# palash1992/GEM

Measured on NVIDIA H100. Metric: nodes/sec embedded at d=128, higher is better.
Workload: dtype f32

## Files before the change

### gem_b200/csrc/common.cuh

```cuda
#pragma once
#include <cuda_runtime.h>
#include <stdint.h>
#include <stdio.h>
#include <string>
#include <vector>
#include "../../include/gemb200.h"

namespace gemb {

void set_error(const char *fmt, ...);
void count_launch(int k = 1);

#define GEMB_CUDA(call)                                                                       \
    do {                                                                                      \
        cudaError_t _e = (call);                                                              \
        if (_e != cudaSuccess) {                                                              \
            gemb::set_error("%s failed at %s:%d: %s", #call, __FILE__, __LINE__,              \
                            cudaGetErrorString(_e));                                          \
            (void)cudaGetLastError();           \
            return GEMB_ERR_CUDA;                                                             \
        }                                                                                     \
    } while (0)

#define GEMB_TRY(call)                                                                        \
// ... 51 lines not shown
    float ms(int from, int to) const { float t = 0.f; cudaEventElapsedTime(&t, ev_[from], ev_[to]); return t; }

  private:
    cudaEvent_t ev_[N] = {};
};

struct Timer {
    std::vector<cudaEvent_t> ev;
    size_t used = 0;
    int begin(cudaStream_t s);
    int end(cudaStream_t s);
    double total_ms();
    void reset() { used = 0; }
    void destroy();
};

}

struct gemb_halo_pool {
    size_t cap_floats = 0;
    int nbuf = 0;
    float *buf[8] = {};
    float *peer_buf[8][8] = {};
    unsigned long long *flags = nullptr;
    unsigned long long *peer_flags[8] = {};
    unsigned long long epoch = 0;
    int *timeout_flag = nullptr;
};

struct gemb_ctx {
    int device = 0;
    int sm_count = 132;
    cudaStream_t stream = nullptr;
    int rank = 0, nranks = 1;
    void *comm = nullptr;
    float *spmm_scratch = nullptr;
    size_t spmm_scratch_bytes = 0;
    double *red_scratch = nullptr;
    size_t red_scratch_bytes = 0;
    gemb::Timer t_spmm, t_dense, t_comm, t_misc;
    gemb_halo_pool halo_pool;
};

struct gemb_csr_dev {
    int64_t nnz = 0;
    int32_t *indptr = nullptr;
    int32_t *indices = nullptr;
    float *data = nullptr;
    int32_t n_heavy = 0, n_items = 0;
    int32_t *heavy_row = nullptr;
    int32_t *heavy_first = nullptr;
    int32_t *item_row = nullptr;
    int32_t *item_beg = nullptr;
};
constexpr int SPMM_HEAVY_DEG = 128, SPMM_HEAVY_CHUNK = 512;

constexpr int GEMB_MAX_RANKS = 8;
constexpr int GEMB_HALO_BUFS = 8;
struct gemb_halo {
    bool ready = false;
    int64_t halo_rows = 0;
    int64_t push_total = 0;
    int32_t *indices_ext = nullptr;
    int32_t *push_ptr = nullptr;
    uint32_t *push_dst = nullptr;
    int nbuf = 0, width = 0;
// ... 22 lines not shown
    bool replicated = false;
    gemb_csr_dev A, AT;
    gemb_halo halo;
};

namespace gemb {

int spmm_launch(gemb_ctx *ctx, const gemb_csr_dev &A, int64_t n_rows, int b, float alpha,
                const float *X, const float *X0, float *Y);
int spmm3_launch(gemb_ctx *ctx, const gemb_csr_dev &A, int64_t n_rows, int b, float alpha, const float *X,
                 float gamma, const float *Xself, float delta, const float *X0, float *Y,
                 const HaloPushArgs *push = nullptr);

int halo_build(gemb_graph *g);
int halo_buffers(gemb_graph *g, int nbuf, int width);
int halo_push_launch(gemb_graph *g, int buf_index, int width);
int halo_barrier(gemb_graph *g);
void halo_push_args(const gemb_graph *g, int buf_index, HaloPushArgs *out);
int halo_free(gemb_graph *g);
void halo_pool_release(gemb_ctx *c);
int halo_check_timeout(gemb_graph *g);

int gram_launch(gemb_ctx *ctx, int64_t n, const float *P, int b1, const float *Q, int b2, double *G);
int apply_launch(gemb_ctx *ctx, int64_t n, const float *Q, int b1, const float *M, int ldm, int b2,
                 float *Out, int ldo);
int apply_fp32_launch(gemb_ctx *ctx, int64_t n, const float *Q, int b1, const float *M, int ldm, int b2,
                      float *Out, int ldo);
int chol_inverse_launch(gemb_ctx *ctx, int b, double *G, float *Minv, int *rank_out_dev, double *Minv64 = nullptr);
int small_gemm_launch(gemb_ctx *ctx, int b, const double *A, int transA, const double *B, double *C, float *C32);
int gram_fp32_launch(gemb_ctx *ctx, int64_t n, const float *P, int b1, const float *Q, int b2, double *G);
int gram_tc_launch(gemb_ctx *ctx, int64_t n, const float *P, int b1, const float *Q, int b2, double *G);
int red_scratch(gemb_ctx *ctx, size_t doubles, double **out);
int sum_partials_launch(gemb_ctx *ctx, int parts, int64_t count, const double *part, double *out);
int eigh_launch(gemb_ctx *ctx, int b, double *G, double *w, double *Z, double *Zscratch , double rel_tol = 1e-11);
int randn_launch(gemb_ctx *ctx, int64_t n, int b, uint64_t seed, uint64_t row_offset, float *X);
int sumsq_launch(gemb_ctx *ctx, int64_t count, const float *X, double *out_dev);
int scale_launch(gemb_ctx *ctx, int64_t count, float s, float *X);
int axpy_launch(gemb_ctx *ctx, int64_t count, float a, const float *X, float *Y);


#ifdef __CUDACC__
__device__ __forceinline__ void halo_push_row(const HaloPushArgs &P, int64_t row, int G, int c, const float4 &r) {
    const int i0 = P.push_ptr[row], i1 = P.push_ptr[row + 1];
    if (i0 == i1) return;
    for (int i = i0; i < i1; i++) {
        const uint32_t d = P.push_dst[i];
        P.peer[d >> 29][(P.halo_row0 + (int64_t)(d & 0x1fffffffu)) * G + c] = r;
    }
}
#endif

}
```

### gem_b200/csrc/core.cu

```cuda
#include "common.cuh"
#include "nccl_api.h"
#include <dlfcn.h>
#include <stdarg.h>
#include <string.h>
#include <atomic>
#include <map>
#include <mutex>
#include <unordered_map>
#include <stdlib.h>

namespace gemb {

static thread_local char g_err[1024] = "";
static std::atomic<long long> g_launches{0};
void count_launch(int k) { g_launches.fetch_add(k, std::memory_order_relaxed); }
long long launches_total() { return g_launches.load(std::memory_order_relaxed); }

void set_error(const char *fmt, ...) {
    va_list ap;
    va_start(ap, fmt);
    vsnprintf(g_err, sizeof g_err, fmt, ap);
    va_end(ap);
}

// ... 158 lines not shown
int gemb_version(void) { return GEMB_VERSION; }
int64_t gemb_launch_count(void) { return (int64_t)gemb::launches_total(); }
const char *gemb_last_error(void) { return g_err; }

int gemb_device_count(void) {
    int n = 0;
    if (cudaGetDeviceCount(&n) != cudaSuccess) {
        cudaGetLastError();
        return 0;
    }
    return n;
}

int gemb_ctx_create(int device, gemb_ctx **out) {
    GEMB_ARG(out != nullptr, "out");
    int n = gemb_device_count();
    if (n <= 0) {
        set_error("no CUDA device visible: libgemb200 has no CPU fallback");
        return GEMB_ERR_CUDA;
    }
    GEMB_ARG(device >= 0 && device < n, "device index");
    GEMB_CUDA(cudaSetDevice(device));
    cudaDeviceProp prop;
    GEMB_CUDA(cudaGetDeviceProperties(&prop, device));
    if (prop.major != 9 || prop.minor != 0) {
        set_error("device %d is sm_%d%d; libgemb200 is built for sm_90a (H100) only", device, prop.major,
                  prop.minor);
        return GEMB_ERR_CUDA;
    }
    gemb_ctx *c = new gemb_ctx();
    c->device = device;
    c->sm_count = prop.multiProcessorCount;
    GEMB_CUDA(cudaStreamCreateWithFlags(&c->stream, cudaStreamNonBlocking));
    *out = c;
    return GEMB_OK;
}

int gemb_ctx_destroy(gemb_ctx *c) {
    if (!c) return GEMB_OK;
    cudaSetDevice(c->device);
    gemb::halo_pool_release(c);
    if (c->comm) {
        NcclApi *api = nccl_api();
        if (api) api->CommDestroy((ncclComm_t)c->comm);
    }
    c->t_spmm.destroy();
    c->t_dense.destroy();
    c->t_comm.destroy();
    c->t_misc.destroy();
    dfree(c->spmm_scratch);
    dfree(c->red_scratch);
    if (c->stream) cudaStreamDestroy(c->stream);
    delete c;
    return GEMB_OK;
}

int gemb_host_alloc(size_t bytes, void **out) {
    GEMB_ARG(out != nullptr, "out");
    GEMB_CUDA(cudaHostAlloc(out, bytes ? bytes : 1, cudaHostAllocDefault));
    return GEMB_OK;
}
int gemb_host_free(void *p) {
    if (p) GEMB_CUDA(cudaFreeHost(p));
    return GEMB_OK;
}

int gemb_comm_unique_id(void *id_out) {
    GEMB_ARG(id_out != nullptr, "id_out");
    NcclApi *api = nccl_api();
    if (!api) return GEMB_ERR_NCCL;
    ncclUniqueId id;
    ncclResult_t r = api->GetUniqueId(&id);
    if (r != ncclSuccess) {
        set_error("ncclGetUniqueId: %s", api->GetErrorString(r));
        return GEMB_ERR_NCCL;
    }
    static_assert(sizeof(id) == GEMB_UNIQUE_ID_BYTES, "ncclUniqueId size");
    memcpy(id_out, &id, sizeof id);
    return GEMB_OK;
}

int gemb_comm_init(gemb_ctx *c, int rank, int nranks, const void *idp) {
    GEMB_ARG(c && idp, "ctx/id");
    GEMB_ARG(nranks >= 1 && rank >= 0 && rank < nranks, "rank/nranks");
    NcclApi *api = nccl_api();
// ... 155 lines not shown
```

### gem_b200/csrc/dense.cu

```cuda
#include "common.cuh"
#include <algorithm>

namespace gemb {

template <int TM>
__global__ void __launch_bounds__(256)
gram_kernel(int64_t n, const float *__restrict__ P, int b1, const float *__restrict__ Q, int b2,
            double *__restrict__ Gpart, int tiles_n) {
    constexpr int BT = 16 * TM;
    constexpr int KC = 32;
    __shared__ float sP[KC][BT];
    __shared__ float sQ[KC][BT];
    const int tid = threadIdx.x;
    const int tx = tid & 15, ty = tid >> 4;
    const int tile_m = blockIdx.y / tiles_n, tile_n = blockIdx.y % tiles_n;
    const int m0 = tile_m * BT, n0 = tile_n * BT;
    float acc[TM][TM];
#pragma unroll
    for (int i = 0; i < TM; i++)
#pragma unroll
        for (int j = 0; j < TM; j++) acc[i][j] = 0.f;

    for (int64_t r0 = (int64_t)blockIdx.x * KC; r0 < n; r0 += (int64_t)gridDim.x * KC) {
        for (int idx = tid; idx < KC * BT; idx += 256) {
// ... 286 lines not shown
        double v = 0.0;
        if (r == c) { v = ldiag[r] > 0.0 ? dscale[r] / ldiag[r] : 0.0; }
        else if (r < c) v = G[r * ld + c] * dscale[r];
        Minv[idx] = (float)v;
        if (Minv64) Minv64[idx] = v;
    }
    if (tid == 0 && rank_out) {
        for (int j = 0; j < b; j++) rank += ldiag[j] > 0.0;
        *rank_out = rank;
    }
}

int chol_inverse_launch(gemb_ctx *ctx, int b, double *G, float *Minv, int *rank_out_dev, double *Minv64) {
    const size_t vecs = sizeof(double) * 3 * (size_t)b;
    const size_t smem = vecs + sizeof(double) * (size_t)b * (b | 1);
    static int optin = 0;
    if (!optin) {
        int v = 0;
        GEMB_CUDA(cudaDeviceGetAttribute(&v, cudaDevAttrMaxSharedMemoryPerBlockOptin, ctx->device));
        GEMB_CUDA(cudaFuncSetAttribute(chol_inverse_kernel<true>, cudaFuncAttributeMaxDynamicSharedMemorySize, v));
        optin = v;
    }
    if (smem <= (size_t)optin) chol_inverse_kernel<true><<<1, 1024, smem, ctx->stream>>>(b, G, Minv, Minv64, rank_out_dev);
    else chol_inverse_kernel<false><<<1, 1024, vecs, ctx->stream>>>(b, G, Minv, Minv64, rank_out_dev);
    GEMB_CUDA(cudaGetLastError());
    count_launch();
    return GEMB_OK;
}

enum JacobiStore { JAC_SHARED, JAC_ZT_GLOBAL, JAC_GLOBAL };
template <JacobiStore STORE>
__global__ void __launch_bounds__(1024)
eigh_jacobi_kernel(int b, double *Ag, double *__restrict__ w, double *__restrict__ Z, double *Ztg, int max_sweeps,
                   double rel_tol) {
    constexpr bool A_GLOBAL = STORE == JAC_GLOBAL, ZT_GLOBAL = STORE != JAC_SHARED;
    extern __shared__ __align__(16) unsigned char sh_fast[];
    double *sh = (double *)sh_fast;
    const int m = (b + 1) & ~1;
    const int half = m / 2;
    const int ld = A_GLOBAL ? b : (b | 1);
    double2 *csn = (double2 *)sh;
    int2 *pq = (int2 *)(sh + 2 * half);
    double *A = A_GLOBAL ? Ag : sh + 3 * half + 2;
    double *ZT = ZT_GLOBAL ? Ztg : A + (size_t)b * ld;
    const int ldz = ZT_GLOBAL ? b : ld;
    __shared__ double s_woff[32], s_wdiag[32];
    const int tid = threadIdx.x, nt = blockDim.x;
    const double *__restrict__ Ain = Ag;
    for (int idx = tid; idx < b * b; idx += nt) {
        const int i = idx / b, j = idx - i * b;
        if (!A_GLOBAL) A[i * ld + j] = Ain[idx];
        ZT[i * ldz + j] = (i == j) ? 1.0 : 0.0;
    }
    const int zb_i0 = tid / b, zb_k0 = tid - zb_i0 * b, zb_di = nt / b, zb_dk = nt - zb_di * b;
    const int bl_i0 = tid / half, bl_j0 = tid - bl_i0 * half, bl_di = nt / half, bl_dj = nt - bl_di * half;
    __syncthreads();
    for (int sweep = 0; sweep < max_sweeps; sweep++) {
        __syncthreads();
        double off = 0.0, dg = 0.0;
        for (int i = zb_i0, j = zb_k0; i < b;) {
            const double v = A[i * ld + j];
            if (i == j) dg += v * v; else off += v * v;
            j += zb_dk; i += zb_di;
            if (j >= b) { j -= b; i++; }
        }
        for (int o = 16; o > 0; o >>= 1) {
            off += __shfl_xor_sync(0xffffffffu, off, o);
            dg += __shfl_xor_sync(0xffffffffu, dg, o);
        }
        if ((tid & 31) == 0) { s_woff[tid >> 5] = off; s_wdiag[tid >> 5] = dg; }
        __syncthreads();
        double s_off = 0.0, s_diag = 0.0;
        for (int w = 0; w < (nt >> 5); w++) { s_off += s_woff[w]; s_diag += s_wdiag[w]; }
        if (s_off <= rel_tol * rel_tol * (s_diag + s_off) || s_diag + s_off == 0.0) break;
        for (int r = 0; r < m - 1; r++) {
            if (tid < half) {
                int p, q;
                if (tid == 0) { p = m - 1; q = r % (m - 1); }
                else { p = (r + tid) % (m - 1); q = (r + m - 1 - tid) % (m - 1); }
                if (p > q) { int t = p; p = q; q = t; }
                double c = 1.0, s = 0.0;
                if (q < b) {
                    const double apq = A[p * ld + q];
                    if (apq != 0.0) {
// ... 60 lines not shown
                }
            } else {
                for (int pi = zb_i0, k = zb_k0; pi < half;) {
                    const double2 rt = csn[pi];
                    const int2 a = pq[pi];
                    if (a.y >= 0 && rt.y != 0.0) {
                        double *xp = ZT + a.x * ldz + k, *yp = ZT + a.y * ldz + k;
                        const double x = *xp, y = *yp;
                        *xp = rt.x * x - rt.y * y;
                        *yp = rt.y * x + rt.x * y;
                    }
                    k += zb_dk; pi += zb_di;
                    if (k >= b) { k -= b; pi++; }
                }
            }
            __syncthreads();
        }
    }
    __syncthreads();
    const int lane = tid & 31, warp = tid >> 5, nwarps = nt >> 5;
    for (int j = warp; j < b; j += nwarps) {
        const double wj = A[j * ld + j];
        int rank = 0;
        for (int i = lane; i < b; i += 32) {
            const double wi = A[i * ld + i];
            rank += (wi < wj) || (wi == wj && i < j);
        }
        for (int o = 16; o > 0; o >>= 1) rank += __shfl_xor_sync(0xffffffffu, rank, o);
        if (lane == 0) w[rank] = wj;
        for (int k = lane; k < b; k += 32) Z[(size_t)k * b + rank] = ZT_GLOBAL ? __ldcg(ZT + j * ldz + k) : ZT[j * ldz + k];
    }
}

int eigh_launch(gemb_ctx *ctx, int b, double *G, double *w, double *Z, double *Zscratch, double rel_tol) {
    const int half = ((b + 1) & ~1) / 2;
    const size_t base = sizeof(double) * (3 * half + 2);
    const size_t cap = 220 * 1024;
    const size_t mat = sizeof(double) * (size_t)b * (b | 1);
    static bool attr_set = false;
    if (!attr_set) {
        GEMB_CUDA(cudaFuncSetAttribute(eigh_jacobi_kernel<JAC_SHARED>, cudaFuncAttributeMaxDynamicSharedMemorySize, (int)cap));
        GEMB_CUDA(cudaFuncSetAttribute(eigh_jacobi_kernel<JAC_ZT_GLOBAL>, cudaFuncAttributeMaxDynamicSharedMemorySize, (int)cap));
        attr_set = true;
    }
    if (base + 2 * mat <= cap) eigh_jacobi_kernel<JAC_SHARED><<<1, 1024, base + 2 * mat, ctx->stream>>>(b, G, w, Z, Zscratch, 30, rel_tol);
    else if (base + mat <= cap) eigh_jacobi_kernel<JAC_ZT_GLOBAL><<<1, 1024, base + mat, ctx->stream>>>(b, G, w, Z, Zscratch, 30, rel_tol);
    else eigh_jacobi_kernel<JAC_GLOBAL><<<1, 1024, base, ctx->stream>>>(b, G, w, Z, Zscratch, 30, rel_tol);
    GEMB_CUDA(cudaGetLastError());
    count_launch();
    return GEMB_OK;
}

__global__ void __launch_bounds__(1024)
small_gemm_kernel(int b, const double *__restrict__ A, int transA, const double *__restrict__ B,
                  double *__restrict__ C, float *__restrict__ C32) {
    for (int idx = threadIdx.x; idx < b * b; idx += blockDim.x) {
        const int i = idx / b, j = idx - i * b;
        double acc = 0.0;
        if (transA) for (int k = 0; k < b; k++) acc += A[(size_t)k * b + i] * B[(size_t)k * b + j];
        else for (int k = 0; k < b; k++) acc += A[(size_t)i * b + k] * B[(size_t)k * b + j];
        if (C) C[idx] = acc;
        if (C32) C32[idx] = (float)acc;
    }
}

int small_gemm_launch(gemb_ctx *ctx, int b, const double *A, int transA, const double *B, double *C, float *C32) {
    small_gemm_kernel<<<1, 1024, 0, ctx->stream>>>(b, A, transA, B, C, C32);
    GEMB_CUDA(cudaGetLastError());
    count_launch();
    return GEMB_OK;
}

__device__ __forceinline__ uint64_t splitmix64(uint64_t x) {
    x += 0x9E3779B97F4A7C15ull;
    x = (x ^ (x >> 30)) * 0xBF58476D1CE4E5B9ull;
    x = (x ^ (x >> 27)) * 0x94D049BB133111EBull;
    return x ^ (x >> 31);
}

__global__ void randn_kernel(int64_t n, int b, uint64_t seed, uint64_t row_offset, float *__restrict__ X) {
// ... 167 lines not shown
```

### gem_b200/csrc/hope.cu

```cuda
#include "common.cuh"
#include <chrono>
#include "nccl_api.h"
#include <math.h>
#include <string.h>
#include <algorithm>
#include <numeric>

namespace gemb {

struct HopeWork {
    gemb_graph *g;
    gemb_ctx *c;
    int b;
    int64_t rows;
    int64_t shard;
    float *buf[5] = {nullptr, nullptr, nullptr, nullptr, nullptr};
    DeviceBuffer<float> own_buf[5];
    DeviceBuffer<float> full;
    DeviceBuffer<double> G, G2, w, Z, Zs, scal;
    DeviceBuffer<float> Minv, M1, M2;
    DeviceBuffer<int> rank_dev;
    int64_t spmm_wide = 0, spmm_all = 0;
    bool halo = false;
    int64_t pushes = 0;
    double push_bytes_per_row = 0.0;
    int buf_index(const float *p) const { for (int i = 0; i < 5; i++) if (buf[i] == p) return i; return -1; }
    int alloc_blocks(size_t count) {
        for (int i = 0; i < 5; i++) {
            GEMB_CUDA(own_buf[i].alloc(count));
            buf[i] = own_buf[i].get();
            GEMB_CUDA(cudaMemsetAsync(buf[i], 0, sizeof(float) * count, c->stream));
        }
        return GEMB_OK;
    }
};

struct HopeResult {
    int iters = 0, converged = 0, katz_terms = 0, algorithm = 0;
    double change = 0.0;
    float resid_max = -1.f, resid_est = -1.f;
    float *Xd = nullptr;
    DeviceBuffer<float> Xalloc;
    float *sig_dev = nullptr;
    double sigma_max = 0.0;
};

static int copy_sync(gemb_ctx *c, void *dst, const void *src, size_t bytes, cudaMemcpyKind kind) {
    GEMB_CUDA(cudaMemcpyAsync(dst, src, bytes, kind, c->stream));
    GEMB_CUDA(cudaStreamSynchronize(c->stream));
    return GEMB_OK;
}

static int clear_scratch(HopeWork &W) {
    for (int i = 2; i < 5; i++) GEMB_CUDA(cudaMemsetAsync(W.buf[i], 0, sizeof(float) * (size_t)W.shard * W.b, W.c->stream));
// ... 125 lines not shown

__global__ void ritz_maps_kernel(int b, int k, const double *__restrict__ w, const double *__restrict__ Z,
                                 float *__restrict__ M1, float *__restrict__ M2, double p1, double p2,
                                 double rel_floor = 1e-28) {
    const int idx = blockIdx.x * blockDim.x + threadIdx.x;
    if (idx >= b * k) return;
    const int i = idx / k, j = idx - i * k;
    const double wmax = w[b - 1];
    const double th = w[b - k + j];
    const double z = Z[(size_t)i * b + (b - k + j)];
    double a = 0.0, c = 0.0;
    if (th > rel_floor * wmax && th > 0.0) { a = z * pow(th, p1); c = z * pow(th, p2); }
    M1[idx] = (float)a;
    M2[idx] = (float)c;
}

__global__ void sqrt_top_kernel(int b, int k, const double *__restrict__ w, float *__restrict__ sigma) {
    const int j = blockIdx.x * blockDim.x + threadIdx.x;
    if (j < k) { const double th = w[b - k + j]; sigma[j] = (float)(th > 0.0 ? sqrt(th) : 0.0); }
}

__global__ void coldiff_sumsq_kernel(int64_t n, int b, const float *__restrict__ A, const float *__restrict__ B,
                                     double *__restrict__ out) {
    const int j = threadIdx.x % b;
    const int rpb = blockDim.x / b;
    double acc = 0.0;
    for (int64_t r = (int64_t)blockIdx.x * rpb + threadIdx.x / b; r < n; r += (int64_t)gridDim.x * rpb) {
        const double d = (double)A[r * b + j] - (double)B[r * b + j];
        acc += d * d;
    }
    atomicAdd(out + j, acc);
}

__global__ void symmetrize_kernel(int b, double *__restrict__ T) {
    const int idx = blockIdx.x * blockDim.x + threadIdx.x;
    if (idx >= b * b) return;
    const int i = idx / b, j = idx - i * b;
    if (i < j) {
        const double v = 0.5 * (T[(size_t)i * b + j] + T[(size_t)j * b + i]);
        T[(size_t)i * b + j] = v;
        T[(size_t)j * b + i] = v;
    }
}

__global__ void axpby_kernel(int64_t count, float a, const float4 *__restrict__ P, float c,
                             const float4 *__restrict__ Q, float4 *__restrict__ Y) {
    for (int64_t i = (int64_t)blockIdx.x * blockDim.x + threadIdx.x; i < count; i += (int64_t)gridDim.x * blockDim.x) {
        const float4 p = P[i], q = Q[i];
        Y[i] = make_float4(a * p.x + c * q.x, a * p.y + c * q.y, a * p.z + c * q.z, a * p.w + c * q.w);
    }
}

__global__ void __launch_bounds__(256)
axpby_push_kernel(int64_t n_rows, int G, int rows_per_cta, float a, const float4 *__restrict__ P, float c,
                  const float4 *__restrict__ Q, float4 *__restrict__ Y, HaloPushArgs H) {
    const int lr = threadIdx.x / G, cc = threadIdx.x - lr * G;
    if (lr >= rows_per_cta) return;
    const int64_t row = (int64_t)blockIdx.x * rows_per_cta + lr;
    if (row >= n_rows) return;
    const float4 p = P[row * G + cc], q = Q[row * G + cc];
    const float4 v = make_float4(a * p.x + c * q.x, a * p.y + c * q.y, a * p.z + c * q.z, a * p.w + c * q.w);
    Y[row * G + cc] = v;
    halo_push_row(H, row, G, cc, v);
}

static int axpby_launch(HopeWork &W, float a, const float *P, float c, const float *Q, float *Y) {
    const int64_t count = W.rows * (int64_t)W.b / 4;
    if (W.halo) {
        const int G = W.b / 4, rpc = 256 / G, bo = W.buf_index(Y);
        GEMB_ARG(bo >= 0 && G <= 256, "axpby output is not a work block");
        HaloPushArgs H;
        halo_push_args(W.g, bo, &H);
        if (W.rows > 0) {
            axpby_push_kernel<<<(unsigned)((W.rows + rpc - 1) / rpc), 256, 0, W.c->stream>>>(
// ... 120 lines not shown
    int oversample = 16, max_iters = 30, min_iters = 2, katz_terms = 0, compute_residual = 0, verbose = 0;
    int algorithm = 0, cheb_degree = 8, stop_rule = 0, lanczos_basis = 0;
    int spectral_mode = 0;
    float tol = 1e-6f, katz_tol = 1e-7f, range_log2 = 8.f;
    uint64_t seed = 1234;
};

static int katz_terms_for(double beta, double nrm, double katz_tol) {
    const double x1 = beta * nrm * 1.02;
    if (x1 <= 1e-30) return 1;
    int J = (int)ceil(log(katz_tol) / log(x1));
    return std::max(1, std::min(J, 4096));
}

static int residual_check(HopeWork &W, float beta, int J, const float *P, const float *Qs, float *scr0, float *scr1,
                          float *scr2, const std::vector<int> &cols, double smax, float *out) {
    gemb_ctx *c = W.c;
    const int b = W.b;
    GEMB_TRY(katz(W, true, beta, J, P, scr0, scr1, scr2));
    GEMB_CUDA(cudaMemsetAsync(W.scal.get(), 0, sizeof(double) * b, c->stream));
    const int threads = (256 / b) * b > 0 ? (256 / b) * b : b;
    coldiff_sumsq_kernel<<<c->sm_count * 4, threads, 0, c->stream>>>(W.rows, b, scr0, Qs, W.scal.get());
    GEMB_CUDA(cudaGetLastError());
    count_launch();
    GEMB_TRY(comm_allreduce_f64(W, W.scal.get(), b));
    std::vector<double> rs(b);
    GEMB_TRY(copy_sync(c, rs.data(), W.scal.get(), sizeof(double) * b, cudaMemcpyDeviceToHost));
    double rm = 0.0;
    for (int j : cols) rm = std::max(rm, sqrt(rs[j]) / std::max(smax, 1e-300));
    *out = (float)rm;
    return GEMB_OK;
}

static int ritz_eigh(HopeWork &W, float tol, std::vector<double> &lam) {
    gemb_ctx *c = W.c;
    const int b = W.b;
    GEMB_TRY(c->t_dense.begin(c->stream));
    GEMB_TRY(eigh_launch(c, b, W.G2.get(), W.w.get(), W.Z.get(), W.Zs.get(), std::min(1e-5, std::max(1e-13, 1e-2 * (double)tol))));
    GEMB_TRY(c->t_dense.end(c->stream));
    return copy_sync(c, lam.data(), W.w.get(), sizeof(double) * b, cudaMemcpyDeviceToHost);
}

static double sigma_change(const double *theta, const double *theta_prev, int k, double tmax) {
    double change = 0.0;
    for (int j = 0; j < k; j++) {
        const double sj = sqrt(std::max(theta[j], 0.0)), sp = sqrt(std::max(theta_prev[j], 0.0));
        change = std::max(change, fabs(sj - sp) / std::max(sj, 1e-3 * sqrt(tmax)));
    }
    return change;
}

static int hope_general(HopeWork &W, const Opts &o, int d, float beta, int J, HopeResult &R) {
    gemb_ctx *c = W.c;
    const int b = W.b, k = d / 2;
    float *V = W.buf[0], *U = W.buf[1], *Wk = W.buf[2], *T1 = W.buf[3], *T2 = W.buf[4];
    R.algorithm = 1;
    R.katz_terms = J;
    GEMB_TRY(randn_launch(c, W.rows, b, o.seed, (uint64_t)W.g->row0, T1));
    GEMB_TRY(cholqr2(W, T1, T2, V));

    std::vector<double> theta(b), theta_prev(b, 0.0);
    for (int it = 1; it <= o.max_iters; it++) {
        R.iters = it;
        GEMB_TRY(katz(W, false, beta, J, V, U, T1, T2));
        GEMB_TRY(gram_full(W, U, U, W.G.get()));
        GEMB_CUDA(cudaMemcpyAsync(W.G2.get(), W.G.get(), sizeof(double) * b * b, cudaMemcpyDeviceToDevice, c->stream));
        GEMB_TRY(ritz_eigh(W, o.tol, theta));
        const double tmax = std::max(theta[b - 1], 1e-300);
        const double change = sigma_change(&theta[b - k], &theta_prev[b - k], k, tmax);
        R.change = change;
        theta_prev = theta;
        if (o.verbose)
            fprintf(stderr, "[gemb_hope/general] it %d  sigma_max %.6g sigma_k %.6g  ritz change %.3g\n", it,
                    sqrt(tmax), sqrt(std::max(theta[b - k], 0.0)), change);
        if (it >= o.min_iters && change <= (double)o.tol) { R.converged = 1; break; }
        if (it == o.max_iters) break;
        GEMB_TRY(c->t_dense.begin(c->stream));
        ritz_maps_kernel<<<(b * b + 255) / 256, 256, 0, c->stream>>>(b, b, W.w.get(), W.Z.get(), W.M1.get(), W.M2.get(), -0.5, 0.5, 1e-10);
        GEMB_CUDA(cudaGetLastError());
        count_launch();
        GEMB_TRY(apply_launch(c, W.rows, U, b, W.M1.get(), b, b, T1, b));
        GEMB_TRY(c->t_dense.end(c->stream));
        GEMB_TRY(katz(W, true, beta, J, T1, Wk, U, T2));
        GEMB_TRY(cholqr2(W, Wk, T1, V));
    }
    R.sigma_max = sqrt(std::max(theta[b - 1], 0.0));

    GEMB_TRY(place_output(W, R, T1, d));
    GEMB_TRY(c->t_dense.begin(c->stream));
    ritz_maps_kernel<<<(b * k + 255) / 256, 256, 0, c->stream>>>(b, k, W.w.get(), W.Z.get(), W.M1.get(), W.M2.get(), -0.25, 0.25);
    GEMB_CUDA(cudaGetLastError());
    count_launch();
    GEMB_TRY(apply_launch(c, W.rows, U, b, W.M1.get(), k, k, R.Xd, d));
    GEMB_TRY(apply_launch(c, W.rows, V, b, W.M2.get(), k, k, R.Xd + k, d));
    sqrt_top_kernel<<<(k + 127) / 128, 128, 0, c->stream>>>(b, k, W.w.get(), R.sig_dev);
    GEMB_CUDA(cudaGetLastError());
    count_launch();
    GEMB_TRY(c->t_dense.end(c->stream));

    if (o.compute_residual) {
// ... 106 lines not shown
static int hope_symmetric(HopeWork &W, const Opts &o, int d, SpecMap map, bool ritz_bound, HopeResult &R) {
    gemb_ctx *c = W.c;
    const int mode = o.spectral_mode;
    const int b = W.b, k = mode ? d : d / 2;
    R.algorithm = 2;
    R.katz_terms = 0;
    float *V = W.buf[0], *AV = W.buf[1];
    float *pool[3] = {W.buf[2], W.buf[3], W.buf[4]};

    GEMB_TRY(randn_launch(c, W.rows, b, o.seed, (uint64_t)W.g->row0, pool[0]));
    GEMB_TRY(publish(W, pool[0], b));
    GEMB_TRY(dist_spmm3(W, false, b, 1.f, pool[0], 0.f, false, 1.f, nullptr, pool[1], true, W.halo));
    GEMB_TRY(dist_spmm3(W, false, b, 1.f, pool[1], 0.f, false, 1.f, nullptr, pool[2], true, W.halo));
    GEMB_TRY(dist_spmm(W, false, b, 1.f, pool[2], nullptr, AV, true));
    GEMB_TRY(gram_full(W, AV, AV, W.G.get()));
    GEMB_TRY(cholqr_pass(W, W.G.get(), AV, pool[0]));
    int rank1 = b;
    GEMB_TRY(copy_sync(c, &rank1, W.rank_dev.get(), sizeof(int), cudaMemcpyDeviceToHost));
    if (rank1 >= b) {
        GEMB_TRY(gram_full(W, pool[0], pool[0], W.G.get()));
        GEMB_TRY(cholqr_pass(W, W.G.get(), pool[0], V));
        GEMB_TRY(publish(W, V, b));
    } else {
        GEMB_TRY(randn_launch(c, W.rows, b, o.seed, (uint64_t)W.g->row0, pool[0]));
        GEMB_TRY(cholqr2(W, pool[0], pool[1], V));
        GEMB_TRY(publish(W, V, b));
        for (int s = 0; s < 3; s++) {
            GEMB_TRY(dist_spmm(W, false, b, 1.f, V, nullptr, AV, true));
            GEMB_TRY(cholqr2(W, AV, pool[0], V));
            GEMB_TRY(publish(W, V, b));
        }
    }

    std::vector<double> lam(b), gval(b), th_sorted(b), th_prev(b, 0.0);
    std::vector<double> Wh(o.stop_rule == 1 ? (size_t)b * b : 0), Zr(o.stop_rule == 1 ? (size_t)b * b : 0);
    std::vector<int> order(b);

    auto run_filter = [&](int deg, double e, double c0, double sigma1, float **out) -> int {
        double sigma = sigma1;
        const double tau2 = 2.0 / sigma1;
        float *prev = V, *cur = pool[0];
        float *free_a = pool[1], *free_b = pool[2];
        GEMB_TRY(axpby_launch(W, (float)(sigma / e), AV, (float)(-sigma * c0 / e), V, cur));
        for (int i = 2; i <= deg; i++) {
            const double sn = 1.0 / (tau2 - sigma);
            float *nxt = free_a;
            GEMB_TRY(dist_spmm3(W, false, b, (float)(2.0 * sn / e), cur, (float)(-2.0 * sn * c0 / e), true,
                                (float)(-sigma * sn), prev, nxt, true, i < deg));
            sigma = sn;
            float *old_prev = prev;
            prev = cur;
            cur = nxt;
            if (old_prev == V) { free_a = free_b; free_b = nullptr; }
            else { free_a = old_prev; }
        }
        *out = cur;
        return GEMB_OK;
    };

    for (int it = 1; it <= o.max_iters; it++) {
        R.iters = it;
        GEMB_TRY(dist_spmm(W, false, b, 1.f, V, nullptr, AV, true));
        GEMB_TRY(gram_full(W, V, AV, W.G2.get()));
        symmetrize_kernel<<<(b * b + 255) / 256, 256, 0, c->stream>>>(b, W.G2.get());
        GEMB_CUDA(cudaGetLastError());
        count_launch();
        GEMB_TRY(ritz_eigh(W, o.tol, lam));
        if (ritz_bound) map.tighten(lam.data(), b, 1.05);
        for (int i = 0; i < b; i++) gval[i] = map.key(lam[i]);
        std::iota(order.begin(), order.end(), 0);
        std::sort(order.begin(), order.end(), [&](int a, int c2) { return gval[a] > gval[c2]; });
        for (int i = 0; i < b; i++) th_sorted[i] = gval[order[i]] * gval[order[i]];
        const double tmax = std::max(th_sorted[0], 1e-300);
        const double change = sigma_change(th_sorted.data(), th_prev.data(), k, tmax);
        R.change = change;
        th_prev = th_sorted;
        if (it == 1 && !mode && o.algorithm == 0 && W.g->n >= 2048 && gval[order[k - 1]] < 0.33 * gval[order[0]] &&
            gval[order[std::min(b - 1, 3)]] < 0.7 * gval[order[0]])
            return GEMB_SWITCH_TO_LANCZOS;
        double stop_measure = change;
        if (o.stop_rule == 1) {
            GEMB_TRY(gram_full(W, AV, AV, W.G.get()));
            GEMB_CUDA(cudaMemcpyAsync(Wh.data(), W.G.get(), sizeof(double) * b * b, cudaMemcpyDeviceToHost, c->stream));
            GEMB_TRY(copy_sync(c, Zr.data(), W.Z.get(), sizeof(double) * b * b, cudaMemcpyDeviceToHost));
            double worst = 0.0;
            for (int j = 0; j < k; j++) {
                const int col = order[j];
                double q = 0.0;
                for (int r = 0; r < b; r++) {
                    double t = 0.0;
                    for (int s2 = 0; s2 < b; s2++) t += Wh[(size_t)r * b + s2] * Zr[(size_t)s2 * b + col];
                    q += Zr[(size_t)r * b + col] * t;
                }
                const double r2 = std::max(q - lam[col] * lam[col], 0.0);
                worst = std::max(worst, map.slope(lam[col]) * sqrt(r2) / std::max(gval[order[0]], 1e-300));
            }
            stop_measure = worst;
            R.resid_est = (float)worst;
        }
        if (o.verbose)
            fprintf(stderr, "[gemb_hope/symmetric] it %d  sigma_max %.6g sigma_k %.6g  ritz change %.3g%s%.3g\n", it,
                    gval[order[0]], gval[order[k - 1]], change, o.stop_rule == 1 ? "  residual " : " ", o.stop_rule == 1 ? stop_measure : 0.0);
        if (it >= o.min_iters && stop_measure <= (double)o.tol) { R.converged = 1; break; }
        if (it == o.max_iters) break;

        const SpecMap::Interval iv = map.damped(lam[order[0]], lam[order[b - 1]]);
        const double sigma1 = iv.e / (iv.aL - iv.c0);
        const double xL = fabs(iv.aL - iv.c0) / iv.e;
        const double growth = xL + sqrt(std::max(xL * xL - 1.0, 0.0));
        int deg = o.cheb_degree;
        if (growth > 1.0 + 1e-9) deg = std::min(deg, (int)floor(log(2.0 * exp2((double)o.range_log2)) / log(growth)));

        if (deg < 2) {
            GEMB_TRY(orth_rotated(W, AV, pool[0], V));
            GEMB_TRY(refill_dropped(W, V, pool[0], pool[1], o.seed + 7919ull * (uint64_t)it));
            GEMB_TRY(publish(W, V, b));
            continue;
        }
        float *filtered = nullptr;
        GEMB_TRY(run_filter(deg, iv.e, iv.c0, sigma1, &filtered));
        float *tmp = nullptr;
        for (float *cand : {pool[0], pool[1], pool[2], AV})
            if (cand != filtered) { tmp = cand; break; }
        GEMB_TRY(orth_rotated(W, filtered, tmp, V));
        GEMB_TRY(refill_dropped(W, V, tmp, filtered, o.seed + 7919ull * (uint64_t)it));
        GEMB_TRY(publish(W, V, b));
    }

    std::vector<double> Zh((size_t)b * b);
    GEMB_TRY(copy_sync(c, Zh.data(), W.Z.get(), sizeof(double) * b * b, cudaMemcpyDeviceToHost));
    std::vector<float> M1((size_t)b * k), M2((size_t)b * k), sig(k);
    std::vector<int> sel(k);
    for (int j = 0; j < k; j++) {
        const int col = order[j], q = map.out_col(j, k);
        const SpecMap::Column t = map.column(lam[col]);
        sel[q] = col;
        sig[q] = (float)t.sigma;
        for (int i = 0; i < b; i++) {
            const double z = Zh[(size_t)i * b + col];
            M2[(size_t)i * k + q] = (float)(z * t.scale);
            M1[(size_t)i * k + q] = (float)((t.neg ? -z : z) * t.scale);
        }
    }
    R.sigma_max = gval[order[0]];
    GEMB_TRY(place_output(W, R, pool[0], d));
    GEMB_CUDA(cudaMemcpyAsync(W.M1.get(), M1.data(), sizeof(float) * b * k, cudaMemcpyHostToDevice, c->stream));
    GEMB_CUDA(cudaMemcpyAsync(W.M2.get(), M2.data(), sizeof(float) * b * k, cudaMemcpyHostToDevice, c->stream));
    GEMB_TRY(copy_sync(c, R.sig_dev, sig.data(), sizeof(float) * k, cudaMemcpyHostToDevice));
    GEMB_TRY(c->t_dense.begin(c->stream));
    GEMB_TRY(apply_launch(c, W.rows, V, b, W.M1.get(), k, k, R.Xd, d));
    if (!mode) GEMB_TRY(apply_launch(c, W.rows, V, b, W.M2.get(), k, k, R.Xd + k, d));
    GEMB_TRY(c->t_dense.end(c->stream));
    if (mode || !o.compute_residual) return GEMB_OK;

    const int J = katz_terms_for(map.beta, ritz_bound ? map.bound / 1.02 : map.norm, o.katz_tol);
    std::vector<float> MP((size_t)b * b, 0.f), MQ((size_t)b * b, 0.f);
    for (int col = 0; col < b; col++) {
        const SpecMap::Column t = map.column(lam[col]);
        for (int i = 0; i < b; i++) {
            const double z = Zh[(size_t)i * b + col];
            MP[(size_t)i * b + col] = (float)(t.neg ? -z : z);
            MQ[(size_t)i * b + col] = (float)(z * t.sigma);
        }
    }
    DeviceBuffer<float> dMP, dMQ, Palloc, Q, STP;
    const size_t blk = (size_t)W.shard * b;
    GEMB_CUDA(dMP.alloc(b * b));
    GEMB_CUDA(dMQ.alloc(b * b));
    float *P = AV;
    if (!W.halo) {
        GEMB_CUDA(Palloc.alloc(blk));
        GEMB_CUDA(cudaMemsetAsync(Palloc.get(), 0, sizeof(float) * blk, c->stream));
        P = Palloc.get();
    }
    GEMB_CUDA(Q.alloc(blk));
    GEMB_CUDA(STP.alloc(blk));
    GEMB_CUDA(cudaMemsetAsync(Q.get(), 0, sizeof(float) * blk, c->stream));
    GEMB_CUDA(cudaMemsetAsync(STP.get(), 0, sizeof(float) * blk, c->stream));
    GEMB_CUDA(cudaMemcpyAsync(dMP.get(), MP.data(), sizeof(float) * b * b, cudaMemcpyHostToDevice, c->stream));
    GEMB_CUDA(cudaMemcpyAsync(dMQ.get(), MQ.data(), sizeof(float) * b * b, cudaMemcpyHostToDevice, c->stream));
    GEMB_TRY(apply_launch(c, W.rows, V, b, dMP.get(), b, b, P, b));
    GEMB_TRY(apply_launch(c, W.rows, V, b, dMQ.get(), b, b, Q.get(), b));
    GEMB_TRY(publish(W, P, b));
    return residual_check(W, (float)map.beta, J, P, Q.get(), STP.get(), W.halo ? pool[1] : AV, W.halo ? pool[2] : pool[1], sel,
// ... 360 lines not shown

    static const bool trace = getenv("GEMB_TRACE") != nullptr;
    auto now = [] { return std::chrono::duration<double, std::milli>(std::chrono::steady_clock::now().time_since_epoch()).count(); };
    const double t_enter = now();
    HopeWork W;
    W.g = g; W.c = c; W.b = b; W.rows = g->n_local; W.shard = g->n_shard;
    static const bool mg_allgather = getenv("GEMB_MG") && !strcmp(getenv("GEMB_MG"), "allgather");
    if (c->nranks > 1 && algo >= 2 && !mg_allgather) {
        int hs = halo_build(g);
        if (hs == GEMB_OK) hs = halo_buffers(g, 5, b);
        NcclApi *api = nccl_api();
        if (!api) return GEMB_ERR_NCCL;
        int hflag = (hs == GEMB_OK) ? 1 : 0;
        DeviceBuffer<int> flag;
        GEMB_CUDA(flag.alloc(1));
        GEMB_CUDA(cudaMemcpyAsync(flag.get(), &hflag, sizeof(int), cudaMemcpyHostToDevice, c->stream));
        ncclResult_t r = api->AllReduce(flag.get(), flag.get(), 1, ncclInt, ncclMin, (ncclComm_t)c->comm, c->stream);
        GEMB_TRY(copy_sync(c, &hflag, flag.get(), sizeof(int), cudaMemcpyDeviceToHost));
        if (r != ncclSuccess) { set_error("ncclAllReduce(halo agreement): %s", api->GetErrorString(r)); return GEMB_ERR_NCCL; }
        W.halo = hflag == 1;
        if (!W.halo && o.verbose) fprintf(stderr, "[gemb_hope] halo exchange unavailable (%s); all-gather per sweep\n", gemb_last_error());
    }
    if (W.halo) {
        for (int i = 0; i < 5; i++) W.buf[i] = g->halo.buf[i];
        GEMB_TRY(halo_barrier(g));
    } else {
        GEMB_TRY(W.alloc_blocks((size_t)W.shard * b));
        if (c->nranks > 1) GEMB_CUDA(W.full.alloc((size_t)g->n_pad * b));
    }
    GEMB_CUDA(W.G.alloc(b * b));
    GEMB_CUDA(W.G2.alloc(b * b));
    GEMB_CUDA(W.Z.alloc(b * b));
    GEMB_CUDA(W.Zs.alloc(b * b));
    GEMB_CUDA(W.w.alloc(b));
    GEMB_CUDA(W.scal.alloc(b + 8));
    GEMB_CUDA(W.Minv.alloc(b * b));
    GEMB_CUDA(W.M1.alloc(b * b));
    GEMB_CUDA(W.M2.alloc(b * b));
    GEMB_CUDA(W.rank_dev.alloc(1));

    c->t_spmm.reset(); c->t_dense.reset(); c->t_comm.reset(); c->t_misc.reset();
    const double t_alloc = now();
    CallEvents<2> ev;
    GEMB_CUDA(ev.create());
    GEMB_CUDA(cudaEventRecord(ev[0], c->stream));

    double nrm = 0.0, hard_bound = 0.0;
    int J = o.katz_terms;
    bool have_nrm = false, ritz_bound = false;
    if (beta < 0.f) {
        GEMB_TRY(estimate_norm2(W, o.seed, W.buf[3], W.buf[4], W.buf[2], &nrm));
        if (!(nrm > 0.0)) { set_error("beta < 0 asks for beta = |beta| / ||A||_2, but ||A||_2 = 0 (empty graph)"); return GEMB_ERR_ARG; }
        beta = (float)(-(double)beta / nrm);
        have_nrm = true;
        GEMB_TRY(clear_scratch(W));
    }
    bool need_power = (J <= 0 && algo == 1) && !have_nrm;
    if (algo >= 2) {
        bool nonneg = false;
        GEMB_TRY(rowsum_bound(W, &hard_bound, &nonneg));
        if (nonneg && (double)beta * hard_bound * 1.02 < 1.0) ritz_bound = true;
        else need_power = !have_nrm;
    }
    if (have_nrm && !ritz_bound) {
        if ((double)beta * nrm * 1.02 >= 1.0) { set_error("|beta| / ||A||_2 with |beta| >= 0.98: outside the Katz convergence radius"); return GEMB_ERR_DIVERGE; }
        if (J <= 0) J = katz_terms_for(beta, nrm, o.katz_tol);
        if (hard_bound <= 0.0) hard_bound = nrm;
    }
    if (need_power) {
        GEMB_TRY(estimate_norm2(W, o.seed, W.buf[3], W.buf[4], W.buf[2], &nrm));
        if ((double)beta * nrm * 1.02 >= 1.0) {
            int Jp = 0;
// ... 83 lines not shown
```

Measured before the change: 18.22 million.

## Overlap AV Gram with eigh on side stream, move Ritz residual to GPU

```diff
diff --git a/gem_b200/csrc/common.cuh b/gem_b200/csrc/common.cuh
--- a/gem_b200/csrc/common.cuh
+++ b/gem_b200/csrc/common.cuh
@@ -107,6 +107,7 @@
     int device = 0;
     int sm_count = 132;
     cudaStream_t stream = nullptr;
+    cudaStream_t side = nullptr;
     int rank = 0, nranks = 1;
     void *comm = nullptr;
     float *spmm_scratch = nullptr;
@@ -195,7 +196,8 @@
 int gram_tc_launch(gemb_ctx *ctx, int64_t n, const float *P, int b1, const float *Q, int b2, double *G);
 int red_scratch(gemb_ctx *ctx, size_t doubles, double **out);
 int sum_partials_launch(gemb_ctx *ctx, int parts, int64_t count, const double *part, double *out);
-int eigh_launch(gemb_ctx *ctx, int b, double *G, double *w, double *Z, double *Zscratch , double rel_tol = 1e-11);
+int eigh_launch(gemb_ctx *ctx, int b, double *G, double *w, double *Z, double *Zscratch , double rel_tol = 1e-11,
+                bool symmetrize = false );
 int randn_launch(gemb_ctx *ctx, int64_t n, int b, uint64_t seed, uint64_t row_offset, float *X);
 int sumsq_launch(gemb_ctx *ctx, int64_t count, const float *X, double *out_dev);
 int scale_launch(gemb_ctx *ctx, int64_t count, float s, float *X);
diff --git a/gem_b200/csrc/core.cu b/gem_b200/csrc/core.cu
--- a/gem_b200/csrc/core.cu
+++ b/gem_b200/csrc/core.cu
@@ -214,6 +214,7 @@
     c->device = device;
     c->sm_count = prop.multiProcessorCount;
     GEMB_CUDA(cudaStreamCreateWithFlags(&c->stream, cudaStreamNonBlocking));
+    GEMB_CUDA(cudaStreamCreateWithFlags(&c->side, cudaStreamNonBlocking));
     *out = c;
     return GEMB_OK;
 }
@@ -233,6 +234,7 @@
     dfree(c->spmm_scratch);
     dfree(c->red_scratch);
     if (c->stream) cudaStreamDestroy(c->stream);
+    if (c->side) cudaStreamDestroy(c->side);
     delete c;
     return GEMB_OK;
 }
diff --git a/gem_b200/csrc/dense.cu b/gem_b200/csrc/dense.cu
--- a/gem_b200/csrc/dense.cu
+++ b/gem_b200/csrc/dense.cu
@@ -342,7 +342,7 @@
 template <JacobiStore STORE>
 __global__ void __launch_bounds__(1024)
 eigh_jacobi_kernel(int b, double *Ag, double *__restrict__ w, double *__restrict__ Z, double *Ztg, int max_sweeps,
-                   double rel_tol) {
+                   double rel_tol, bool symmetrize) {
     constexpr bool A_GLOBAL = STORE == JAC_GLOBAL, ZT_GLOBAL = STORE != JAC_SHARED;
     extern __shared__ __align__(16) unsigned char sh_fast[];
     double *sh = (double *)sh_fast;
@@ -359,7 +359,8 @@
     const double *__restrict__ Ain = Ag;
     for (int idx = tid; idx < b * b; idx += nt) {
         const int i = idx / b, j = idx - i * b;
-        if (!A_GLOBAL) A[i * ld + j] = Ain[idx];
+        if (!A_GLOBAL) A[i * ld + j] = (symmetrize && i != j) ? 0.5 * (Ain[idx] + Ain[j * b + i]) : Ain[idx];
+        else if (symmetrize && i < j) Ag[idx] = Ag[j * b + i] = 0.5 * (Ag[idx] + Ag[j * b + i]);
         ZT[i * ldz + j] = (i == j) ? 1.0 : 0.0;
     }
     const int zb_i0 = tid / b, zb_k0 = tid - zb_i0 * b, zb_di = nt / b, zb_dk = nt - zb_di * b;
@@ -486,7 +487,7 @@
     }
 }
 
-int eigh_launch(gemb_ctx *ctx, int b, double *G, double *w, double *Z, double *Zscratch, double rel_tol) {
+int eigh_launch(gemb_ctx *ctx, int b, double *G, double *w, double *Z, double *Zscratch, double rel_tol, bool symmetrize) {
     const int half = ((b + 1) & ~1) / 2;
     const size_t base = sizeof(double) * (3 * half + 2);
     const size_t cap = 220 * 1024;
@@ -497,9 +498,9 @@
         GEMB_CUDA(cudaFuncSetAttribute(eigh_jacobi_kernel<JAC_ZT_GLOBAL>, cudaFuncAttributeMaxDynamicSharedMemorySize, (int)cap));
         attr_set = true;
     }
-    if (base + 2 * mat <= cap) eigh_jacobi_kernel<JAC_SHARED><<<1, 1024, base + 2 * mat, ctx->stream>>>(b, G, w, Z, Zscratch, 30, rel_tol);
-    else if (base + mat <= cap) eigh_jacobi_kernel<JAC_ZT_GLOBAL><<<1, 1024, base + mat, ctx->stream>>>(b, G, w, Z, Zscratch, 30, rel_tol);
-    else eigh_jacobi_kernel<JAC_GLOBAL><<<1, 1024, base, ctx->stream>>>(b, G, w, Z, Zscratch, 30, rel_tol);
+    if (base + 2 * mat <= cap) eigh_jacobi_kernel<JAC_SHARED><<<1, 1024, base + 2 * mat, ctx->stream>>>(b, G, w, Z, Zscratch, 30, rel_tol, symmetrize);
+    else if (base + mat <= cap) eigh_jacobi_kernel<JAC_ZT_GLOBAL><<<1, 1024, base + mat, ctx->stream>>>(b, G, w, Z, Zscratch, 30, rel_tol, symmetrize);
+    else eigh_jacobi_kernel<JAC_GLOBAL><<<1, 1024, base, ctx->stream>>>(b, G, w, Z, Zscratch, 30, rel_tol, symmetrize);
     GEMB_CUDA(cudaGetLastError());
     count_launch();
     return GEMB_OK;
diff --git a/gem_b200/csrc/hope.cu b/gem_b200/csrc/hope.cu
--- a/gem_b200/csrc/hope.cu
+++ b/gem_b200/csrc/hope.cu
@@ -20,6 +20,7 @@
     DeviceBuffer<double> G, G2, w, Z, Zs, scal;
     DeviceBuffer<float> Minv, M1, M2;
     DeviceBuffer<int> rank_dev;
+    CallEvents<2> fork_join;
     int64_t spmm_wide = 0, spmm_all = 0;
     bool halo = false;
     int64_t pushes = 0;
@@ -211,14 +212,20 @@
     atomicAdd(out + j, acc);
 }
 
-__global__ void symmetrize_kernel(int b, double *__restrict__ T) {
-    const int idx = blockIdx.x * blockDim.x + threadIdx.x;
-    if (idx >= b * b) return;
-    const int i = idx / b, j = idx - i * b;
-    if (i < j) {
-        const double v = 0.5 * (T[(size_t)i * b + j] + T[(size_t)j * b + i]);
-        T[(size_t)i * b + j] = v;
-        T[(size_t)j * b + i] = v;
+__global__ void ritz_quadform_kernel(int b, const double *__restrict__ H, const double *__restrict__ Z,
+                                     double *__restrict__ q) {
+    extern __shared__ double s_term[];
+    const int col = blockIdx.x;
+    for (int r = threadIdx.x; r < b; r += blockDim.x) {
+        double t = 0.0;
+        for (int s = 0; s < b; s++) t = __dadd_rn(t, __dmul_rn(H[(size_t)r * b + s], Z[(size_t)s * b + col]));
+        s_term[r] = __dmul_rn(Z[(size_t)r * b + col], t);
+    }
+    __syncthreads();
+    if (threadIdx.x == 0) {
+        double acc = 0.0;
+        for (int r = 0; r < b; r++) acc = __dadd_rn(acc, s_term[r]);
+        q[col] = acc;
     }
 }
 
@@ -405,13 +412,28 @@
     return GEMB_OK;
 }
 
-static int ritz_eigh(HopeWork &W, float tol, std::vector<double> &lam) {
+static int ritz_eigh(HopeWork &W, float tol, bool symmetrize, std::vector<double> &lam, const float *AV = nullptr) {
     gemb_ctx *c = W.c;
     const int b = W.b;
     GEMB_TRY(c->t_dense.begin(c->stream));
-    GEMB_TRY(eigh_launch(c, b, W.G2.get(), W.w.get(), W.Z.get(), W.Zs.get(), std::min(1e-5, std::max(1e-13, 1e-2 * (double)tol))));
+    if (AV) GEMB_CUDA(cudaEventRecord(W.fork_join[0], c->stream));
+    GEMB_TRY(eigh_launch(c, b, W.G2.get(), W.w.get(), W.Z.get(), W.Zs.get(), std::min(1e-5, std::max(1e-13, 1e-2 * (double)tol)),
+                         symmetrize));
+    if (AV) {
+        GEMB_CUDA(cudaStreamWaitEvent(c->side, W.fork_join[0], 0));
+        std::swap(c->stream, c->side);
+        const int s = gram_launch(c, W.rows, AV, b, AV, b, W.G.get());
+        std::swap(c->stream, c->side);
+        GEMB_TRY(s);
+        GEMB_CUDA(cudaEventRecord(W.fork_join[1], c->side));
+        GEMB_CUDA(cudaStreamWaitEvent(c->stream, W.fork_join[1], 0));
+        GEMB_TRY(comm_allreduce_f64(W, W.G.get(), (size_t)b * b));
+        ritz_quadform_kernel<<<b, 128, sizeof(double) * b, c->stream>>>(b, W.G.get(), W.Z.get(), W.w.get() + b);
+        GEMB_CUDA(cudaGetLastError());
+        count_launch();
+    }
     GEMB_TRY(c->t_dense.end(c->stream));
-    return copy_sync(c, lam.data(), W.w.get(), sizeof(double) * b, cudaMemcpyDeviceToHost);
+    return copy_sync(c, lam.data(), W.w.get(), sizeof(double) * (AV ? 2 * b : b), cudaMemcpyDeviceToHost);
 }
 
 static double sigma_change(const double *theta, const double *theta_prev, int k, double tmax) {
@@ -438,7 +460,7 @@
         GEMB_TRY(katz(W, false, beta, J, V, U, T1, T2));
         GEMB_TRY(gram_full(W, U, U, W.G.get()));
         GEMB_CUDA(cudaMemcpyAsync(W.G2.get(), W.G.get(), sizeof(double) * b * b, cudaMemcpyDeviceToDevice, c->stream));
-        GEMB_TRY(ritz_eigh(W, o.tol, theta));
+        GEMB_TRY(ritz_eigh(W, o.tol, false, theta));
         const double tmax = std::max(theta[b - 1], 1e-300);
         const double change = sigma_change(&theta[b - k], &theta_prev[b - k], k, tmax);
         R.change = change;
@@ -611,8 +633,7 @@
         }
     }
 
-    std::vector<double> lam(b), gval(b), th_sorted(b), th_prev(b, 0.0);
-    std::vector<double> Wh(o.stop_rule == 1 ? (size_t)b * b : 0), Zr(o.stop_rule == 1 ? (size_t)b * b : 0);
+    std::vector<double> lam(2 * b), gval(b), th_sorted(b), th_prev(b, 0.0);
     std::vector<int> order(b);
 
     auto run_filter = [&](int deg, double e, double c0, double sigma1, float **out) -> int {
@@ -641,10 +662,7 @@
         R.iters = it;
         GEMB_TRY(dist_spmm(W, false, b, 1.f, V, nullptr, AV, true));
         GEMB_TRY(gram_full(W, V, AV, W.G2.get()));
-        symmetrize_kernel<<<(b * b + 255) / 256, 256, 0, c->stream>>>(b, W.G2.get());
-        GEMB_CUDA(cudaGetLastError());
-        count_launch();
-        GEMB_TRY(ritz_eigh(W, o.tol, lam));
+        GEMB_TRY(ritz_eigh(W, o.tol, true, lam, o.stop_rule == 1 ? AV : nullptr));
         if (ritz_bound) map.tighten(lam.data(), b, 1.05);
         for (int i = 0; i < b; i++) gval[i] = map.key(lam[i]);
         std::iota(order.begin(), order.end(), 0);
@@ -659,19 +677,10 @@
             return GEMB_SWITCH_TO_LANCZOS;
         double stop_measure = change;
         if (o.stop_rule == 1) {
-            GEMB_TRY(gram_full(W, AV, AV, W.G.get()));
-            GEMB_CUDA(cudaMemcpyAsync(Wh.data(), W.G.get(), sizeof(double) * b * b, cudaMemcpyDeviceToHost, c->stream));
-            GEMB_TRY(copy_sync(c, Zr.data(), W.Z.get(), sizeof(double) * b * b, cudaMemcpyDeviceToHost));
             double worst = 0.0;
             for (int j = 0; j < k; j++) {
                 const int col = order[j];
-                double q = 0.0;
-                for (int r = 0; r < b; r++) {
-                    double t = 0.0;
-                    for (int s2 = 0; s2 < b; s2++) t += Wh[(size_t)r * b + s2] * Zr[(size_t)s2 * b + col];
-                    q += Zr[(size_t)r * b + col] * t;
-                }
-                const double r2 = std::max(q - lam[col] * lam[col], 0.0);
+                const double r2 = std::max(lam[b + col] - lam[col] * lam[col], 0.0);
                 worst = std::max(worst, map.slope(lam[col]) * sqrt(r2) / std::max(gval[order[0]], 1e-300));
             }
             stop_measure = worst;
@@ -708,7 +717,8 @@
 
     std::vector<double> Zh((size_t)b * b);
     GEMB_TRY(copy_sync(c, Zh.data(), W.Z.get(), sizeof(double) * b * b, cudaMemcpyDeviceToHost));
-    std::vector<float> M1((size_t)b * k), M2((size_t)b * k), sig(k);
+    const int xw = mode ? k : 2 * k;
+    std::vector<float> M((size_t)b * xw), sig(k);
     std::vector<int> sel(k);
     for (int j = 0; j < k; j++) {
         const int col = order[j], q = map.out_col(j, k);
@@ -717,18 +727,16 @@
         sig[q] = (float)t.sigma;
         for (int i = 0; i < b; i++) {
             const double z = Zh[(size_t)i * b + col];
-            M2[(size_t)i * k + q] = (float)(z * t.scale);
-            M1[(size_t)i * k + q] = (float)((t.neg ? -z : z) * t.scale);
+            M[(size_t)i * xw + q] = (float)((t.neg ? -z : z) * t.scale);
+            if (!mode) M[(size_t)i * xw + k + q] = (float)(z * t.scale);
         }
     }
     R.sigma_max = gval[order[0]];
     GEMB_TRY(place_output(W, R, pool[0], d));
-    GEMB_CUDA(cudaMemcpyAsync(W.M1.get(), M1.data(), sizeof(float) * b * k, cudaMemcpyHostToDevice, c->stream));
-    GEMB_CUDA(cudaMemcpyAsync(W.M2.get(), M2.data(), sizeof(float) * b * k, cudaMemcpyHostToDevice, c->stream));
+    GEMB_CUDA(cudaMemcpyAsync(W.M1.get(), M.data(), sizeof(float) * b * xw, cudaMemcpyHostToDevice, c->stream));
     GEMB_TRY(copy_sync(c, R.sig_dev, sig.data(), sizeof(float) * k, cudaMemcpyHostToDevice));
     GEMB_TRY(c->t_dense.begin(c->stream));
-    GEMB_TRY(apply_launch(c, W.rows, V, b, W.M1.get(), k, k, R.Xd, d));
-    if (!mode) GEMB_TRY(apply_launch(c, W.rows, V, b, W.M2.get(), k, k, R.Xd + k, d));
+    GEMB_TRY(apply_launch(c, W.rows, V, b, W.M1.get(), xw, xw, R.Xd, d));
     GEMB_TRY(c->t_dense.end(c->stream));
     if (mode || !o.compute_residual) return GEMB_OK;
 
@@ -1155,12 +1163,13 @@
     GEMB_CUDA(W.G2.alloc(b * b));
     GEMB_CUDA(W.Z.alloc(b * b));
     GEMB_CUDA(W.Zs.alloc(b * b));
-    GEMB_CUDA(W.w.alloc(b));
+    GEMB_CUDA(W.w.alloc(2 * b));
     GEMB_CUDA(W.scal.alloc(b + 8));
     GEMB_CUDA(W.Minv.alloc(b * b));
-    GEMB_CUDA(W.M1.alloc(b * b));
+    GEMB_CUDA(W.M1.alloc((size_t)b * std::max(b, d)));
     GEMB_CUDA(W.M2.alloc(b * b));
     GEMB_CUDA(W.rank_dev.alloc(1));
+    GEMB_CUDA(W.fork_join.create());
 
     c->t_spmm.reset(); c->t_dense.reset(); c->t_comm.reset(); c->t_misc.reset();
     const double t_alloc = now();
```

Result: faster. 19.00 million, median of 6 (+4.3%).
